# lyuchenyang/Macaw-LLM

Measured on AMD Instinct MI355X. Metric: multimodal samples/sec (img+audio+128 tok) fwd+bwd at 1/2/4/8 MI355X, higher is better.
Workload: dtype bf16; 1 GPU; BASELINE cfg 3: CLIP-ViT-L/14 + Whisper-base + LLaMA-7B, image + 30 s audio + 128-token text (S=144); fwd+bwd+fused AdamW, encoders frozen as run_clm_llms.py:390-393, alignment-attention dropout on; global_batch=32, per_gpu_batch=32, seq_len=144, parallelism=dp1: 20 flat buckets, 13476 MiB of parameters, local (one fused AdamW launch), step_launch=eager, kernel by kernel, grad_weight_side_stream=off (engine.DW_SIDE auto), setup_steps=1, activation_checkpointing=False

## Files before the change

macaw_llm_amd/build.py:

```python
from __future__ import annotations

import hashlib
import os
import shutil
import subprocess
import sys
from concurrent.futures import ThreadPoolExecutor
from pathlib import Path

PKG = Path(__file__).resolve().parent
CSRC = PKG / "csrc"
OBJ = PKG / "csrc" / "_obj"
LIB = PKG / "libmacaw_hip.so"
ARCH = "gfx950"
EXPERIMENTS = bool(os.environ.get("MK_EXPERIMENTS"))
SOURCES = ["gemm.hip", "gemm_v7.hip", *(["gemm_v8.hip"] if EXPERIMENTS else []), "gemm_v9.hip", "norm.hip",
           "elementwise.hip", "softmax.hip", "attention.hip", "decode.hip", "decode_fp8.hip", "decode_mxfp4.hip", "sample.hip", "logits_process.hip", "beam.hip", "spec.hip", "logprobs.hip", "cfg.hip", "preprocess.hip", "lora.hip"]
FLAGS = ["-O3", "-std=c++17", "-fPIC", f"--offload-arch={ARCH}", "-fno-gpu-rdc", *os.environ.get("MK_EXTRA_FLAGS", "").split(),
         *(["-DMK_WITH_V8", "-DMK_WITH_FWD4X64"] if EXPERIMENTS else []), "-Wno-unused-result"]


FILE_FLAGS = {"gemm_v8.hip": ["-mllvm", "-pragma-unroll-threshold=1000000"],
              "gemm_v9.hip": ["-mllvm", "-pragma-unroll-threshold=1000000"]}


def _hipcc() -> str:
    for cand in (os.environ.get("HIPCC"), shutil.which("hipcc"), "/opt/rocm/bin/hipcc"):
        if cand and Path(cand).exists():
            return cand
    raise RuntimeError("hipcc not found: cannot build libmacaw_hip.so")


def _digest(paths) -> str:
    h = hashlib.sha256()
    for p in sorted(paths):
        h.update(p.name.encode())
        h.update(p.read_bytes())
    h.update(" ".join(FLAGS).encode())
    h.update(repr(sorted(FILE_FLAGS.items())).encode())
    return h.hexdigest()


def build(force: bool = False, verbose: bool = True) -> Path:
    srcs = [CSRC / s for s in SOURCES]
    deps = srcs + [CSRC / "common.h", CSRC / "gemm_common.h", CSRC / "gemm_group_plan.h", PKG.parent / "include" / "macaw_hip.h",
                   *sorted(CSRC.glob("*.inc"))]
    stamp = OBJ / "stamp.txt"
    dig = _digest(deps)
    if not force and LIB.exists() and stamp.exists() and stamp.read_text() == dig:
        return LIB
    OBJ.mkdir(parents=True, exist_ok=True)
    hipcc = _hipcc()

    def compile_one(src: Path) -> Path:
        obj = OBJ / (src.stem + ".o")
        cmd = [hipcc, *FLAGS, *FILE_FLAGS.get(src.name, []), "-c", str(src), "-o", str(obj)]
        r = subprocess.run(cmd, capture_output=True, text=True)
        if r.returncode != 0:
            raise RuntimeError(f"hipcc failed for {src.name}:\n{r.stderr[-4000:]}")
        return obj

    with ThreadPoolExecutor(max_workers=min(8, len(srcs))) as ex:
        objs = list(ex.map(compile_one, srcs))
    cmd = [hipcc, "-shared", "-fPIC", f"--offload-arch={ARCH}", "-o", str(LIB), *map(str, objs)]
    r = subprocess.run(cmd, capture_output=True, text=True)
    if r.returncode != 0:
        raise RuntimeError(f"link failed:\n{r.stderr[-4000:]}")
    stamp.write_text(dig)
    if verbose:
        print(f"[macaw_llm_amd.build] built {LIB} ({LIB.stat().st_size/1e6:.1f} MB)", file=sys.stderr)
    return LIB


if __name__ == "__main__":
    build(force="--force" in sys.argv)
```

macaw_llm_amd/csrc/gemm.hip:

```cpp
#include "common.h"
#include "../../include/macaw_hip.h"
#include "gemm_common.h"
#include "gemm_group_plan.h"
#include <cstdio>
#include <algorithm>
#include <cstdlib>
#include <utility>
#include <vector>

namespace {
using namespace mkg;

constexpr int BM = 128, BN = 128, BK = 64;
#ifndef MK_GEMM_DEFAULT_CFG
#define MK_GEMM_DEFAULT_CFG 5
#endif
constexpr int TILE_BYTES = 128 * 64 * 2;
}

#define MK_E16_T bf16
#define MK_E16_NS e_bf16
#include "gemm_impl.inc"
#undef MK_E16_T
#undef MK_E16_NS
#define MK_E16_T _Float16
#define MK_E16_NS e_f16
#define gemm_bf16_kernel gemm_f16_kernel
#define gemm_bf16_v2_kernel gemm_f16_v2_kernel
#define gemm_fp8_v2_kernel gemm_fp8_v2_kernel_unused
#include "gemm_impl.inc"
#undef gemm_bf16_kernel
#undef gemm_bf16_v2_kernel
#undef gemm_fp8_v2_kernel
#undef MK_E16_T
#undef MK_E16_NS

namespace {
using namespace mkg;

constexpr int FBM = 64, FBN = 64, FBK = 16, FPAD = 4;

template <bool RED_MAJOR>
MK_DEV void f32_tile_load(const float* base, long ld, int row0, int k0, int R, int K,
                          float (*lds)[FBM + FPAD]) {
  const int t = threadIdx.x;
  if constexpr (!RED_MAJOR) {
    const int row = t >> 2, kq = (t & 3) * 4;
    const int gr = row0 + row;
#pragma unroll
    for (int j = 0; j < 4; ++j) {
      const int gk = k0 + kq + j;
      lds[kq + j][row] = (gr < R && gk < K) ? base[(long)gr * ld + gk] : 0.f;
    }
  } else {
    const int kr = t >> 4, mq = (t & 15) * 4;
    const int gk = k0 + kr;
// ... 177 lines not shown
  return N >= 8192 ? 22 : 19;
}
}

extern "C" int mk_gemm_set_cfg(int cfg) { g_force_cfg = cfg; return MK_OK; }
extern "C" int mk_gemm_has_cfg(int cfg) {
#ifdef MK_WITH_V8
  if (cfg == 14) return 1;
#endif
  return cfg == 0 || cfg == 5 || cfg == 7 || cfg == 11 || cfg == 15;
}
namespace { int g_plan_cus = 0; }
extern "C" int mk_gemm_set_cus(int n) { const int prev = g_plan_cus; g_plan_cus = n > 0 ? n : 0; return prev; }

namespace mkg {
int launch_v7(const GemmArgs& g, bool a_red, bool b_red, dim3 grid, hipStream_t st, bool fp8, bool f16);
#ifdef MK_WITH_V8
int launch_v8(const GemmArgs& g, bool a_red, bool b_red, dim3 grid, hipStream_t st, bool f16);
#endif
int launch_v9(const GemmArgs& g, bool a_red, bool b_red, dim3 grid, hipStream_t st, bool f16);
int v9_mfma16_layouts();
int launch_grp(const GrpArgs& g, bool has_main, int n_wg, hipStream_t st, bool f16);
}

extern "C" int mk_decode_linear(const void* x, int64_t ldx, const void* W, int64_t ldw, void* y,
                                int64_t ldy, const void* residual, int64_t ldr, int32_t M, int32_t N,
                                int32_t K, int32_t prologue, const void* norm_w, float eps,
                                int32_t dtype, void* stream) {
  if (!x || !W || !y || M <= 0 || N <= 0 || K <= 0) return MK_ERR_BAD_ARG;
  if (prologue < 0 || prologue > 2 || (prologue == 1 && !norm_w)) return MK_ERR_BAD_ARG;
  if ((dtype != MK_BF16 && dtype != MK_F16) || M > (prologue ? 16 : 32) || (K % 64) || (ldx % 8) || (ldw % 8) ||
      !aligned16(x) || !aligned16(W) || (prologue == 1 && !aligned16(norm_w)))
    return MK_ERR_UNSUPPORTED;
  GemmArgs g{};
  g.A = x; g.B = W; g.C = y; g.R = residual;
  g.M = M; g.N = N; g.K = K;
  g.lda = ldx; g.ldb = ldw; g.ldc = ldy; g.ldr = ldr;
  g.alpha = 1.f;
  g.pro_w = norm_w; g.pro_eps = eps;
  hipStream_t st = reinterpret_cast<hipStream_t>(stream);
  const bool wide = N <= 16 * 256 && K <= 4096;
  const size_t lds = prologue ? (size_t)M * (K + 8) * 2 : 0;
  if (lds > 40 * 1024) return MK_ERR_UNSUPPORTED;
  const int prof = mkp::begin(st, 0, 2.0 * M * N * K, M, N, K, 1, 0, 17 + 10 * prologue);
  if (M > 16) {
    if (dtype == MK_F16) e_f16::launch_skinny(g, skinny32_cfg(N), N, st);
    else e_bf16::launch_skinny(g, skinny32_cfg(N), N, st);
  } else if (dtype == MK_F16) e_f16::launch_decode_linear(g, N, prologue, wide, lds, st);
  else e_bf16::launch_decode_linear(g, N, prologue, wide, lds, st);
  mkp::end(prof, st);
  return mk_check_launch();
}
namespace {
int pick_cfg(const mk_gemm_desc* d, int nbatch, bool v7_ok, int n_cus) {
  static const bool no_v7 = getenv("MK_GEMM_NO_V7") != nullptr;
  if (!v7_ok || no_v7 || nbatch != 1) return MK_GEMM_DEFAULT_CFG;
  const int layout = (d->a_red_major ? 2 : 0) + (d->b_red_major ? 1 : 0);
  const double nk = (d->K + 63) / 64;
  const long T7 = (long)mk_cdiv(d->M, 256) * mk_cdiv(d->N, 256);
  const long full = T7 / n_cus, R = T7 % n_cus;
  const double a7 = layout == 3 ? 1.53 : layout == 1 ? 1.51 : layout == 2 ? 1.52 : 1.46;
  const double tile7 = nk * a7 + 11.5, sub7 = nk * 0.48 + 7.0;
  double t7 = full * tile7;
  if (R > 0) t7 += (4 * R <= 2 * n_cus) ? (double)mk_cdiv((int)(4 * R), n_cus) * sub7
                                         : nk * a7 * (0.55 + 0.45 * R / n_cus) + 11.5;
  const long T2 = (long)mk_cdiv(d->M, 128) * mk_cdiv(d->N, 128);
  const long slots2 = (long)n_cus * (layout == 3 ? 4 : 2);
  const double tile2 = layout == 3 ? nk * 2.18 + 4.0 : nk * (layout == 0 ? 1.67 : 1.45) + 2.0;
  const double a2 = layout == 3 ? 2.18 : layout == 0 ? 1.67 : 1.45;
  const double nk2 = layout == 3 ? 2 * nk : nk;
  double t2;
  if (T2 < slots2) {
    double sp = (double)(slots2 / T2);
    if (sp > nk2 / 2) sp = nk2 / 2;
    if (sp > 64) sp = 64;
    if (sp < 1) sp = 1;
    const double alone = sp > 1 ? 1.0 : 0.57 + 0.43 * std::min(1.0, std::max(0.0, (double)T2 / n_cus - 1.0));
    t2 = nk / sp * a2 * alone + 2.0 + (sp > 1 ? 4.0 + 1.6 * sp : 0.0);
  } else {
    t2 = (double)T2 / slots2 * tile2;
    if (const long R2 = T2 % slots2) {
      double sp = (double)slots2 / R2;
      if (sp > nk2 / 2) sp = nk2 / 2;
      if (sp > 64) sp = 64;
      t2 += 4.0 + 0.65 * sp;
    }
  }
  if (!(t7 * 0.95 < t2)) return MK_GEMM_DEFAULT_CFG;
  static const int v9_mode = [] { const char* e = getenv("MK_GEMM_V9"); return e ? atoi(e) : 1; }();
  const bool m16 = ((mkg::v9_mfma16_layouts() >> layout) & 1) != 0;
  const bool v9_legal = d->dtype != MK_F32 && d->dtype != MK_FP8 && d->M % 256 == 0 && d->N % 256 == 0 && d->K % 64 == 0 &&
                        full >= 1 && !d->scale_a && !d->scale_b &&
                        d->bias_mode == 0 && d->act == 0 && !d->accumulate && (m16 || !d->R);
  const bool nt16 = m16 && layout == 0 && !(R > 0 && full < 2 && nk < 128);
  if (v9_legal && (v9_mode == 2 || (v9_mode == 1 && (layout == 3 || layout == 1 || nk >= 256 || nt16)))) return 15;
  return 11;
}
}

extern "C" int mk_abi_version(void) { return MK_ABI_VERSION; }

extern "C" int mk_gemm(const mk_gemm_desc* d_in, void* stream) {
  const mk_gemm_desc* d = d_in;
  if (!d || !d->A || !d->B || !d->C) return MK_ERR_BAD_ARG;
  if (d->M <= 0 || d->N <= 0 || d->K <= 0) return MK_ERR_BAD_ARG;
  if (d->nb1 < 1 || d->nb2 < 1) return MK_ERR_BAD_ARG;
  if (d->bias_mode && !d->bias) return MK_ERR_BAD_ARG;
  mk_gemm_desc dd;
  bool fp8 = false;
  if (d->dtype == MK_FP8) {
    if (d->a_red_major || d->b_red_major || (d->K % 128) || (d->lda % 16) || (d->ldb % 16) ||
        (d->sA1 % 16) || (d->sA2 % 16) || (d->sB1 % 16) || (d->sB2 % 16) || !aligned16(d->A) ||
        !aligned16(d->B))
      return MK_ERR_UNSUPPORTED;
    dd = *d;
    dd.K /= 2; dd.lda /= 2; dd.ldb /= 2;
    dd.sA1 /= 2; dd.sA2 /= 2; dd.sB1 /= 2; dd.sB2 /= 2;
    dd.dtype = MK_BF16;
    d = &dd;
    fp8 = true;
  }
  if (d->dtype != MK_F32 && d->dtype != MK_BF16 && d->dtype != MK_F16) return MK_ERR_UNSUPPORTED;
  const bool f16 = d->dtype == MK_F16;
  const bool e16 = d->dtype == MK_BF16 || f16;
  GemmArgs g;
  g.scale_a = d->scale_a; g.scale_b = d->scale_b;
  g.scale_vec = (d->flags & MK_GEMM_SCALE_VEC) ? 1 : 0;
  if (g.scale_vec && (!d->scale_a || !d->scale_b)) return MK_ERR_BAD_ARG;
  if (g.scale_vec && !fp8) return MK_ERR_UNSUPPORTED;
  g.A = d->A; g.B = d->B; g.C = d->C; g.R = d->R; g.bias = d->bias;
  g.M = d->M; g.N = d->N; g.K = d->K;
  g.lda = d->lda; g.ldb = d->ldb; g.ldc = d->ldc; g.ldr = d->ldr;
  g.nb2 = d->nb2;
  g.sA1 = d->sA1; g.sA2 = d->sA2; g.sB1 = d->sB1; g.sB2 = d->sB2;
  g.sC1 = d->sC1; g.sC2 = d->sC2; g.sR1 = d->sR1; g.sR2 = d->sR2;
  g.alpha = d->alpha; g.bias_mode = d->bias_mode; g.act = d->act; g.accumulate = d->accumulate;
  hipStream_t st = reinterpret_cast<hipStream_t>(stream);
  const int nbatch = d->nb1 * d->nb2;
  const int prof = mkp::begin(st, fp8 ? 3 : 0, 2.0 * d->M * d->N * d->K * nbatch * (fp8 ? 2 : 1), d->M, d->N,
                              d->K * (fp8 ? 2 : 1), nbatch, d->a_red_major * 2 + d->b_red_major, -1);
  static const int skinny_max = [] { const char* e = getenv("MK_GEMM_SKINNY_MAX_M"); return e ? atoi(e) : 32; }();
  if (e16 && !fp8 && d->M <= 32 && d->M <= skinny_max && !d->a_red_major && !d->b_red_major && nbatch == 1 &&
      (d->K % 64) == 0 && (d->lda % 8) == 0 && (d->ldb % 8) == 0 && aligned16(d->A) && aligned16(d->B) &&
      !getenv("MK_GEMM_NO_SKINNY")) {
    int sk = d->M <= 16 ? ((d->N <= 16 * 256 && d->K <= 4096) ? 18 : 17) : skinny32_cfg(d->N);
    if ((g_force_cfg == 12 || g_force_cfg == 19 || g_force_cfg == 22) ||
        ((g_force_cfg == 13 || g_force_cfg == 17 || g_force_cfg == 18) && d->M <= 16)) sk = g_force_cfg;
// ... 28 lines not shown
      (void)hipGetDevice(&dev);
      (void)hipDeviceGetAttribute(&cus, hipDeviceAttributeMultiprocessorCount, dev);
      return cus;
    }();
    const int n_cus = (g_plan_cus > 0 && g_plan_cus < dev_cus) ? g_plan_cus : dev_cus;
    int cfg;
    if (env_cfg >= 0) cfg = env_cfg;
    else cfg = pick_cfg(d, nbatch, v7_ok, n_cus);
    if (fp8 && cfg != 11) cfg = 5;
#ifndef MK_WITH_V8
    if (cfg == 14) cfg = 11;
#endif
    if ((cfg == 11 || cfg == 14 || cfg == 15) && !v7_ok) cfg = 5;
    if ((cfg == 14 || cfg == 15) && fp8) cfg = 11;
    if (cfg == 15 && (d->M % 256 != 0 || d->N % 256 != 0 || d->K % 64 != 0 || d->K < 128)) cfg = 11;
    if (cfg == 15 && ((mkg::v9_mfma16_layouts() >> ((d->a_red_major ? 2 : 0) + (d->b_red_major ? 1 : 0))) & 1) &&
        (d->bias_mode != 0 || d->act != 0 || d->accumulate || d->scale_a || d->scale_b))
      cfg = 11;
    if (cfg != 0 && cfg != 5 && cfg != 7 && cfg != 11 && cfg != 14 && cfg != 15) cfg = 5;
    if (cfg >= 5 && !v2_ok) cfg = 0;
    if (fp8 && cfg != 5 && cfg != 11) return MK_ERR_UNSUPPORTED;
    if (cfg == 5 && d->a_red_major && d->b_red_major && !getenv("MK_GEMM_NO_BK32")) cfg = 7;
    const int bkv = cfg == 7 ? 32 : BK;
    mkp::set_cfg(prof, cfg);
    const bool v8 = cfg == 14;
    const bool v9 = cfg == 15;
    const bool t256 = cfg == 11 || v8 || v9;
    const int bm = t256 ? 256 : 128;
    const int bn = t256 ? 256 : BN;
    g.tiles_m = mk_cdiv(d->M, bm);
    g.tiles_n = mk_cdiv(d->N, bn);
    g.a_vec = aligned16(d->A) && (d->lda % 8 == 0) && (d->sA1 % 8 == 0) && (d->sA2 % 8 == 0);
    g.b_vec = aligned16(d->B) && (d->ldb % 8 == 0) && (d->sB1 % 8 == 0) && (d->sB2 % 8 == 0);
    const auto c_aligned = [&](uintptr_t mask, long q) {
      return ((reinterpret_cast<uintptr_t>(d->C) & mask) == 0) && (d->ldc % q == 0) && (d->sC1 % q == 0) &&
             (d->sC2 % q == 0) &&
             (!d->R || (((reinterpret_cast<uintptr_t>(d->R) & mask) == 0) && (d->ldr % q == 0) &&
                        (d->sR1 % q == 0) && (d->sR2 % q == 0)));
    };
    g.c_vec = c_aligned(15, 8) ? 2 : c_aligned(7, 4) ? 1 : 0;
    dim3 grid(g.tiles_m * g.tiles_n, 1, nbatch);
    g.dp_tiles = g.tiles_m * g.tiles_n;
    g.lin_batch = 0;
    g.split = 1;
    g.kt_per_piece = 0;
    g.ws = nullptr;
    g.counters = nullptr;
    g.ablate = 0;
    {
      static const int v9_lds_epi = getenv("MK_V9_LDS_EPI") ? 1 : 0;
      if (cfg == 15 && v9_lds_epi) g.ablate = 9;
    }
    g.tail8 = 0;
    const int slots = n_cus * (t256 ? 1 : (cfg == 7 ? 4 : 2));
    static const bool no_streamk = getenv("MK_GEMM_NO_STREAMK") != nullptr;
    if (t256 && !v8 && !no_streamk) {
      const int T = g.tiles_m * g.tiles_n, R = T % n_cus;
      static const bool no_tail8 = getenv("MK_GEMM_NO_TAIL8") != nullptr;
      if (R > 0 && 8 * R <= n_cus && !d->a_red_major && !no_tail8) {
        g.dp_tiles = T - R;
        g.tail8 = 1;
        grid.x = g.dp_tiles + 8 * R;
      } else if (R > 0 && 4 * R <= 2 * n_cus) {
        g.dp_tiles = T - R;
        grid.x = g.dp_tiles + 4 * R;
      }
    } else if ((cfg == 5 || cfg == 7) && d->ws && !no_streamk) {
      const int T = g.tiles_m * g.tiles_n * nbatch, nkt = (d->K + bkv - 1) / bkv;
      const int R = T % slots;
      int sp = R > 0 ? slots / R : 1;
      if (sp > nkt / 2) sp = nkt / 2;
      if (sp > 64) sp = 64;
      const long need = 4096 + (long)R * sp * (64 * 256) * 4;
      if (R > 0 && sp >= 2 && need <= d->ws_bytes) {
        g.dp_tiles = T - R;
        g.split = sp;
        g.kt_per_piece = (nkt + sp - 1) / sp;
        g.counters = reinterpret_cast<int*>(d->ws);
        g.ws = reinterpret_cast<float*>(reinterpret_cast<char*>(d->ws) + 4096);
        if (R * (int)sizeof(int) > 4096) { g.dp_tiles = T; g.split = 1; }
        else {
          grid.x = g.dp_tiles + R * sp;
          if (nbatch > 1) { g.lin_batch = 1; grid.z = 1; }
        }
      }
    }
    g.walkers = g.dp_tiles;
    if (t256 && !v8 && !v9) {
      static const bool no_walk = getenv("MK_GEMM_NO_WALK") != nullptr;
      if (!no_walk && nbatch == 1 && n_cus % 8 == 0 && g.dp_tiles > n_cus && g.dp_tiles % n_cus == 0) {
        grid.x = n_cus + (grid.x - g.dp_tiles);
        g.walkers = n_cus;
      }
    }
#ifdef MK_WITH_V8
    if (v8) {
      const int rc = mkg::launch_v8(g, d->a_red_major != 0, d->b_red_major != 0, grid, st, f16);
      mkp::end(prof, st);
      return rc;
    }
#endif
    const bool v9_c_ok = !((mkg::v9_mfma16_layouts() >> ((d->a_red_major ? 2 : 0) + (d->b_red_major ? 1 : 0))) & 1) || g.c_vec >= 1;
    if (v9 && g.dp_tiles >= n_cus && v9_c_ok) {
      const int tail_wgs = (int)grid.x - g.walkers;
      dim3 gmain(g.dp_tiles, 1, nbatch);
      static const bool no_walk9 = getenv("MK_GEMM_NO_WALK") != nullptr;
      const bool plain9 = d->bias_mode == 0 && d->act == 0 && !d->R && !d->accumulate && g.c_vec == 2 && !d->scale_a &&
                          !d->scale_b && g.ablate != 9;
      const int lay9 = (d->a_red_major ? 2 : 0) + (d->b_red_major ? 1 : 0);
      const bool regepi9 = plain9 || (((mkg::v9_mfma16_layouts() >> lay9) & 1) && g.c_vec >= 1 && d->bias_mode == 0 && d->act == 0 &&
                                      !d->accumulate && !d->scale_a && !d->scale_b && g.ablate != 9);
      if (!no_walk9 && regepi9 && nbatch == 1 && n_cus % 8 == 0 && g.dp_tiles > n_cus && g.dp_tiles % n_cus == 0)
        gmain.x = n_cus;
      int rc = mkg::launch_v9(g, d->a_red_major != 0, d->b_red_major != 0, gmain, st, f16);
      if (rc == MK_OK && tail_wgs > 0) {
        GemmArgs gt = g;
        gt.walkers = 0;
        rc = mkg::launch_v7(gt, d->a_red_major != 0, d->b_red_major != 0, dim3(tail_wgs, 1, nbatch), st, false, f16);
      }
      mkp::end(prof, st);
      return rc;
    }
    if (t256) {
      if (v9) mkp::set_cfg(prof, 11);
      const int rc = mkg::launch_v7(g, d->a_red_major != 0, d->b_red_major != 0, grid, st, fp8, f16);
      mkp::end(prof, st);
      return rc;
    }
    if (f16) (void)e_f16::launch_tile(g, cfg, d->a_red_major != 0, d->b_red_major != 0, false, grid, st);
    else (void)e_bf16::launch_tile(g, cfg, d->a_red_major != 0, d->b_red_major != 0, fp8, grid, st);
  } else {
    g.tiles_m = mk_cdiv(d->M, FBM);
    g.tiles_n = mk_cdiv(d->N, FBN);
    g.a_vec = g.b_vec = g.c_vec = 0;
    dim3 grid(g.tiles_m * g.tiles_n, 1, nbatch), block(256);
    if (!d->a_red_major && !d->b_red_major)
      MK_LAUNCH((gemm_f32_kernel<false, false>), grid, block, 0, st, g);
    else if (!d->a_red_major && d->b_red_major)
      MK_LAUNCH((gemm_f32_kernel<false, true>), grid, block, 0, st, g);
    else if (d->a_red_major && !d->b_red_major)
      MK_LAUNCH((gemm_f32_kernel<true, false>), grid, block, 0, st, g);
    else
      MK_LAUNCH((gemm_f32_kernel<true, true>), grid, block, 0, st, g);
  }
  mkp::end(prof, st);
  return mk_check_launch();
}

extern "C" int mk_gemm_grouped(const mk_gemm_desc* main, mk_gemm_group_fill* fill, int32_t n_fill, int32_t drain,
                               void* stream) {
  static_assert(mkgp::MAX_FILL == GRP_MAX_FILL && mkgp::MAX_WG == GRP_MAX_WG && MK_GROUP_MAX_FILL == GRP_MAX_FILL, "one limit");
  if (n_fill < 0 || (n_fill > 0 && !fill)) return MK_ERR_BAD_ARG;
  for (int i = 0; i < n_fill; ++i) fill[i].taken = 0;
  if (!main && n_fill == 0) return MK_OK;
  if (n_fill > GRP_MAX_FILL || mkg::v9_mfma16_layouts() != 15) return MK_NOT_GROUPED;
  const int dtype = main ? main->dtype : fill[0].d.dtype;
  if (dtype != MK_BF16 && dtype != MK_F16) return MK_NOT_GROUPED;
  const auto member = [&](const mk_gemm_desc& d, int a_red) {
    if (!d.A || !d.B || !d.C || d.M <= 0 || d.N <= 0 || d.K <= 0) return MK_ERR_BAD_ARG;
    const auto span = [&](bool red, long ld) { return red ? (long)d.K * ld * 2 : (256L * ld + d.K) * 2; };
    const bool ok = d.dtype == dtype && d.a_red_major == a_red && d.b_red_major == 1 && d.nb1 == 1 && d.nb2 == 1 &&
                    d.M % 256 == 0 && d.N % 256 == 0 && d.K % 64 == 0 && d.K >= 128 && d.bias_mode == 0 && !d.bias && d.act == 0 &&
                    !d.R && !d.accumulate && !d.scale_a && !d.scale_b && d.flags == 0 && aligned16(d.A) && aligned16(d.B) &&
                    d.lda % 8 == 0 && d.ldb % 8 == 0 && (reinterpret_cast<uintptr_t>(d.C) & 7) == 0 && d.ldc % 4 == 0 &&
                    d.lda >= (a_red ? d.M : d.K) && d.ldb >= d.N && d.ldc >= d.N &&
                    span(a_red != 0, d.lda) < 0x7fffffffL && span(true, d.ldb) < 0x7fffffffL;
// ... 71 lines not shown
```

macaw_llm_amd/csrc/gemm_common.h:

```cpp
#pragma once
#include "common.h"
#include "../../include/macaw_hip.h"

namespace mkg {

struct GemmArgs {
  const void* A; const void* B; void* C; const void* R; const void* bias;
  int M, N, K;
  long lda, ldb, ldc, ldr;
  int nb2;
  long sA1, sA2, sB1, sB2, sC1, sC2, sR1, sR2;
  float alpha;
  const float* scale_a; const float* scale_b;
  int scale_vec;
  int bias_mode, act, accumulate;
  int tiles_m, tiles_n;
  int a_vec, b_vec;
  int c_vec;
  int dp_tiles, split, kt_per_piece;
  int walkers;
  int tail8;
  int lin_batch;
  int ablate;
  const void* pro_w; float pro_eps;
  float* ws;
  int* counters;
};

constexpr int GRP_MAX_FILL = 8, GRP_MAX_WG = 320;
struct GrpProb {
  const void* A; const void* B; void* C;
  long lda, ldb, ldc;
  int M, N, K;
  int tiles_m, tiles_n;
  int first, count;
  float alpha;
};
struct GrpArgs {
  GrpProb p[1 + GRP_MAX_FILL];
  int n_fill;
  int main_tiles;
  unsigned short start[GRP_MAX_WG + 1];
};

MK_DEV float apply_act(float v, int act) {
  if (act == 1) return 0.5f * v * (1.0f + mk_erf(v * 0.70710678118654752440f));
  if (act == 2) return v / (1.0f + __expf(-1.702f * v));
  return v;
}

MK_DEV int xcd_remap(int bid, int nwg) {
  const int xcd = bid & 7;
  const int q = nwg >> 3, r = nwg & 7;
  return (xcd < r ? xcd * (q + 1) : r * (q + 1) + (xcd - r) * q) + (bid >> 3);
}
MK_DEV void tile_from_index(int wg, int tiles_m, int tiles_n, int& tm, int& tn, int GROUP_M);
MK_DEV void tile_coords(int bid, int tiles_m, int tiles_n, int& tm, int& tn) {
  tile_from_index(xcd_remap(bid, tiles_m * tiles_n), tiles_m, tiles_n, tm, tn, 8);
}
MK_DEV void tile_from_index(int wg, int tiles_m, int tiles_n, int& tm, int& tn, int GROUP_M = 8) {
  const int per_group = GROUP_M * tiles_n;
  const int group = wg / per_group;
  const int first_m = group * GROUP_M;
  const int gsize = min(tiles_m - first_m, GROUP_M);
  const int in_g = wg - group * per_group;
  tm = first_m + in_g % gsize;
  tn = in_g / gsize;
}

template <bool SV, typename ET, int FM, int FN>
MK_DEV void wave_epilogue(const f32x16 (&acc)[FM][FN], const GemmArgs& g, ET* C, const ET* Rp,
                          int m0, int n0, int wm0, int wn0, char* smem) {
  typedef typename E16<ET>::x4 e16x4;
  constexpr int W4 = FN * 8;
// ... 249 lines not shown
```

macaw_llm_amd/csrc/gemm_v9.hip:

```cpp
#include "gemm_common.h"
#include "gemm_v9_loop.inc"

#define MK_E16_T bf16
#define MK_E16_NS e_bf16
#define MK_V9_SFX "bf16"
#include "gemm_v9_impl.inc"
#undef MK_E16_T
#undef MK_E16_NS
#undef MK_V9_SFX
#define MK_E16_T _Float16
#define MK_E16_NS e_f16
#define MK_V9_SFX "f16"
#define gemm_bf16_v9_kernel gemm_f16_v9_kernel
#define gemm_bf16_grp_kernel gemm_f16_grp_kernel
#include "gemm_v9_impl.inc"
#undef gemm_bf16_v9_kernel
#undef gemm_bf16_grp_kernel
#undef MK_E16_T
#undef MK_E16_NS
#undef MK_V9_SFX

namespace mkg {
int v9_mfma16_layouts() {
#ifdef V9_MFMA16
  return V9_MFMA16;
#else
  return 0;
#endif
}
int launch_v9(const GemmArgs& g, bool a_red, bool b_red, dim3 grid, hipStream_t st, bool f16) {
  if (f16) {
    if (!a_red && !b_red) return e_f16::launch_v9<false, false>(g, grid, st);
    if (!a_red && b_red) return e_f16::launch_v9<false, true>(g, grid, st);
    if (a_red && !b_red) return e_f16::launch_v9<true, false>(g, grid, st);
    return e_f16::launch_v9<true, true>(g, grid, st);
  }
  if (!a_red && !b_red) return e_bf16::launch_v9<false, false>(g, grid, st);
  if (!a_red && b_red) return e_bf16::launch_v9<false, true>(g, grid, st);
  if (a_red && !b_red) return e_bf16::launch_v9<true, false>(g, grid, st);
  return e_bf16::launch_v9<true, true>(g, grid, st);
}
int launch_grp(const GrpArgs& g, bool has_main, int n_wg, hipStream_t st, bool f16) {
  return f16 ? e_f16::launch_grp(g, has_main, n_wg, st) : e_bf16::launch_grp(g, has_main, n_wg, st);
}
}
```

macaw_llm_amd/csrc/gemm_v9_impl.inc:

```

namespace {
namespace MK_E16_NS {
using namespace mkg;
typedef MK_E16_T e16;
typedef E16<e16>::x8 e16x8;
typedef E16<e16>::x4 e16x4;

constexpr int BM9 = 256, BN9 = 256, BK7 = 64;
constexpr int HALF_BYTES = 128 * BK7 * 2;
constexpr int A_SLOT = 2 * HALF_BYTES;
constexpr int B_BASE9 = 3 * A_SLOT;
constexpr int LDS9 = 5 * A_SLOT;

#include "gemm_lds_image.inc"

typedef uint32_t u32x4 __attribute__((ext_vector_type(4)));

struct V9Tile {
  int m0, n0;
  e16* C;
  const e16* Rp;
  __amdgpu_buffer_rsrc_t rsA, rsB;
  u32x4 dA, dB;
  int voA[2][4], voB[2][4];
// ... 46 lines not shown
  t.dA[3] = 0x00020000u;
  t.dB[0] = __builtin_amdgcn_readfirstlane((uint32_t)pb);
  t.dB[1] = __builtin_amdgcn_readfirstlane((uint32_t)(pb >> 32) & 0xffffu);
  t.dB[2] = (uint32_t)b_rec;
  t.dB[3] = 0x00020000u;
#pragma unroll
  for (int h = 0; h < 2; ++h)
#pragma unroll
    for (int i = 0; i < 4; ++i) {
      t.voA[h][i] = v9_voffset<A_RED, M16>(m0, g.M, g.lda, h, w + 4 * i, l);
      t.voB[h][i] = v9_voffset<B_RED, M16>(n0, g.N, g.ldb, h, w + 4 * i, l);
    }
}

template <typename T>
MK_DEV T* v9_batch_elem(T* p, long z1, long s1, long z2, long s2) {
  return p + z1 * s1 + z2 * s2;
}
template <bool A_RED, bool B_RED>
MK_DEV void v9_tile_setup(const GemmArgs& g, int tile, int w, int l, V9Tile& t) {
  int tm, tn;
  tile_from_index(xcd_remap(tile, g.dp_tiles), g.tiles_m, g.tiles_n, tm, tn, 8);
  const int z = blockIdx.z, z1 = z / g.nb2, z2 = z - z1 * g.nb2;
  const e16* A = v9_batch_elem(reinterpret_cast<const e16*>(g.A), z1, g.sA1, z2, g.sA2);
  const e16* B = v9_batch_elem(reinterpret_cast<const e16*>(g.B), z1, g.sB1, z2, g.sB2);
  t.C = v9_batch_elem(reinterpret_cast<e16*>(g.C), z1, g.sC1, z2, g.sC2);
  t.Rp = g.R ? v9_batch_elem(reinterpret_cast<const e16*>(g.R), z1, g.sR1, z2, g.sR2) : nullptr;
  v9_operand_setup<A_RED, B_RED, true>(g, A, B, tm * BM9, tn * BN9, w, l, t);
}

MK_DEV void v9_tile_request(const V9Tile& t, char* smem, int w, int stepA, int stepB) {
#define V9_DMA_A(DST, H, I, KO)                                                                   \
  __builtin_amdgcn_raw_ptr_buffer_load_lds(                                                       \
      t.rsA, (__attribute__((address_space(3))) void*)(smem + (DST) + (H) * HALF_BYTES + (w + 4 * (I)) * 1024), \
      16, t.voA[H][I], KO, 0, 0)
#define V9_DMA_B(DST, H, I, KO)                                                                   \
  __builtin_amdgcn_raw_ptr_buffer_load_lds(                                                       \
      t.rsB, (__attribute__((address_space(3))) void*)(smem + (DST) + (H) * HALF_BYTES + (w + 4 * (I)) * 1024), \
      16, t.voB[H][I], KO, 0, 0)
#pragma unroll
  for (int h = 0; h < 2; ++h)
#pragma unroll
    for (int i = 0; i < 4; ++i) { V9_DMA_A(0, h, i, 0); V9_DMA_B(B_BASE9, h, i, 0); }
#pragma unroll
  for (int h = 0; h < 2; ++h)
#pragma unroll
    for (int i = 0; i < 4; ++i) V9_DMA_A(A_SLOT, h, i, stepA);
#pragma unroll
  for (int i = 0; i < 4; ++i) V9_DMA_B(B_BASE9 + A_SLOT, 0, i, stepB);
#undef V9_DMA_A
#undef V9_DMA_B
}

#define V9_ASM(TEXT, CLOBBERS)                                                                    \
  asm volatile(TEXT                                                                               \
               :                                                                                  \
               : [voA] "v"(t.voA[0][0]), [voB] "v"(t.voB[0][0]), [adA] "v"(adA), [adB] "v"(adB),   \
                 [rsA] "s"(t.dA), [rsB] "s"(t.dB), [iA] "s"(iA), [iB] "s"(iB), [stA] "s"(stepA),   \
                 [stB] "s"(stepB), [nk] "s"(nk), [wv] "s"(wv)                                      \
               : CLOBBERS)
#if V9_MFMA16
#ifdef MK_V9_NT_STORE
typedef unsigned int v9_u32x2 __attribute__((ext_vector_type(2)));
#define V9_ST8(PTR, VAL) __builtin_nontemporal_store(__builtin_bit_cast(v9_u32x2, VAL), reinterpret_cast<v9_u32x2*>(PTR))
#else
#define V9_ST8(PTR, VAL) (*reinterpret_cast<e16x4*>(PTR) = (VAL))
#endif
#define V9_F16P(I, J, CROW, LDC, ALPHA)                                           \
  do {                                                                                            \
    float t_[4];                                                                                  \
    V9_ACC16_READ_##I##_##J(t_);                                                                  \
    e16x4 o_;                                                                                     \
    _Pragma("unroll") for (int e_ = 0; e_ < 4; ++e_) o_[e_] = (e16)(t_[e_] * (ALPHA));           \
    V9_ST8((CROW) + (long)(16 * (I)) * (LDC) + 16 * (J), o_);                                     \
  } while (0)
#define V9_R16(F, I, CROW, LDC, ALPHA)                                                            \
  do {                                                                                            \
    F(I, 0, CROW, LDC, ALPHA); F(I, 1, CROW, LDC, ALPHA); F(I, 2, CROW, LDC, ALPHA); F(I, 3, CROW, LDC, ALPHA); \
    F(I, 4, CROW, LDC, ALPHA); F(I, 5, CROW, LDC, ALPHA); F(I, 6, CROW, LDC, ALPHA); F(I, 7, CROW, LDC, ALPHA); \
    __builtin_amdgcn_sched_barrier(0);                                                            \
  } while (0)
#define V9_EPI16(F, CROW, LDC, ALPHA)                                                             \
  do {                                                                                            \
    V9_R16(F, 0, CROW, LDC, ALPHA); V9_R16(F, 1, CROW, LDC, ALPHA); V9_R16(F, 2, CROW, LDC, ALPHA); \
    V9_R16(F, 3, CROW, LDC, ALPHA); V9_R16(F, 4, CROW, LDC, ALPHA); V9_R16(F, 5, CROW, LDC, ALPHA); \
    V9_R16(F, 6, CROW, LDC, ALPHA); V9_R16(F, 7, CROW, LDC, ALPHA);                               \
  } while (0)
#endif

template <bool A_RED, bool B_RED>
__global__ __launch_bounds__(256, 1) void gemm_bf16_v9_kernel(GemmArgs g) {
  extern __shared__ __attribute__((aligned(16))) char smem[];
  const int l = threadIdx.x & 63;
  const int w = __builtin_amdgcn_readfirstlane(threadIdx.x >> 6);
  const int wr = w >> 1, wc = w & 1;
  const int wm0 = wr * 128, wn0 = wc * 128;
  const int stepA = A_RED ? (int)(BK7 * g.lda * 2) : BK7 * 2;
  const int stepB = B_RED ? (int)(BK7 * g.ldb * 2) : BK7 * 2;
  const int iA = (int)((A_RED ? 16 : 32) * g.lda * 2);
  const int iB = (int)((B_RED ? 16 : 32) * g.ldb * 2);
  int offA[4], offB[4];
  v7_read_offsets<A_RED>(0, l, offA);
  v7_read_offsets<B_RED>(0, l, offB);
  const int nk = __builtin_amdgcn_readfirstlane((g.K + BK7 - 1) / BK7);
  const uint32_t lds0 = __builtin_amdgcn_readfirstlane(
      (uint32_t)(size_t)((__attribute__((address_space(3))) char*)smem));
  const uint32_t wv = lds0 + (uint32_t)w * 1024u;
  constexpr bool M16 = ((V9_MFMA16 >> (2 * (A_RED ? 1 : 0) + (B_RED ? 1 : 0))) & 1) != 0;
  const uint32_t adA = lds0 + wr * HALF_BYTES + (M16 ? v9_read_offset16<A_RED>(l) : offA[0]);
  const uint32_t adB = lds0 + B_BASE9 + wc * HALF_BYTES + (M16 ? v9_read_offset16<B_RED>(l) : offB[0]);
  const bool plain = g.bias_mode == 0 && g.act == 0 && g.R == nullptr && g.accumulate == 0 && (g.c_vec == 2 || (M16 && g.c_vec >= 1)) &&
                     g.scale_a == nullptr && g.scale_b == nullptr && g.ablate != 9;

  int tile = blockIdx.x;
  const int stride = (int)gridDim.x;
  V9Tile t;
  v9_tile_setup<A_RED, B_RED>(g, tile, w, l, t);
  v9_tile_request(t, smem, w, stepA, stepB);
  bool first = true;
  for (;;) {
    __builtin_amdgcn_sched_barrier(0);
#define V9_LOOPS(W)                                                                               \
  do {                                                                                            \
    if constexpr (!A_RED && !B_RED) V9_ASM(V9_LOOP_TEXT_00##W, V9_LOOP_CLOBBERS);                 \
    else if constexpr (!A_RED && B_RED) V9_ASM(V9_LOOP_TEXT_01##W, V9_LOOP_CLOBBERS);             \
    else if constexpr (A_RED && !B_RED) V9_ASM(V9_LOOP_TEXT_10##W, V9_LOOP_CLOBBERS);             \
    else V9_ASM(V9_LOOP_TEXT_11##W, V9_LOOP_CLOBBERS);                                            \
  } while (0)
#if V9_MFMA16
#define V9_LOOPS16(W)                                                                             \
  do {                                                                                            \
    if constexpr (!A_RED && !B_RED) V9_ASM(V9_LOOP16_TEXT_00##W, V9_LOOP16_CLOBBERS);             \
    else if constexpr (!A_RED && B_RED) V9_ASM(V9_LOOP16_TEXT_01##W, V9_LOOP16_CLOBBERS);         \
    else if constexpr (A_RED && !B_RED) V9_ASM(V9_LOOP16_TEXT_10##W, V9_LOOP16_CLOBBERS);         \
    else V9_ASM(V9_LOOP16_TEXT_11##W, V9_LOOP16_CLOBBERS);                                        \
  } while (0)
    if constexpr (M16) {
      if (first) V9_LOOPS16();
      else V9_LOOPS16(_W);
    } else
#endif
    {
      if (first) V9_LOOPS();
      else V9_LOOPS(_W);
    }
#undef V9_LOOPS
#undef V9_LOOPS16
    __builtin_amdgcn_sched_barrier(0);
#ifdef MK_V9_NOEPI
    return;
#endif
    const int m0 = t.m0, n0 = t.n0;
    e16* C = t.C;
    const e16* Rp = t.Rp;
    const int ntile = tile + stride;
    const bool more = ntile < g.dp_tiles;
    if (more) {
      v9_tile_setup<A_RED, B_RED>(g, ntile, w, l, t);
      __builtin_amdgcn_s_barrier();
      v9_tile_request(t, smem, w, stepA, stepB);
    }
#if V9_MFMA16
    if constexpr (M16) {
      const float alpha = g.alpha;
      const int mrow = m0 + wm0 + (l & 15), ncol = n0 + wn0 + 4 * (l >> 4);
      e16* crow = C + (long)mrow * g.ldc + ncol;
      const e16* rrow = Rp ? Rp + (long)mrow * g.ldr + ncol : nullptr;
#define V9_F16R(I, J, CROW, LDC, ALPHA)    \
  do {                                                                                            \
    float t_[4];                                                                                  \
    V9_ACC16_READ_##I##_##J(t_);                                                                  \
    e16x4 o_;                                                                                     \
    _Pragma("unroll") for (int e_ = 0; e_ < 4; ++e_) o_[e_] = (e16)(t_[e_] * (ALPHA) + (float)rv_[I][J][e_]); \
    V9_ST8((CROW) + (long)(16 * (I)) * (LDC) + 16 * (J), o_);                                     \
  } while (0)
      if (rrow == nullptr) {
        V9_EPI16(V9_F16P, crow, g.ldc, alpha);
      } else {
        e16x4 rv_[8][8];
#pragma unroll
        for (int i_ = 0; i_ < 8; ++i_)
#pragma unroll
          for (int j_ = 0; j_ < 8; ++j_)
            rv_[i_][j_] = *reinterpret_cast<const e16x4*>(rrow + (long)(16 * i_) * g.ldr + 16 * j_);
        __builtin_amdgcn_sched_barrier(0);
        V9_EPI16(V9_F16R, crow, g.ldc, alpha);
      }
#undef V9_F16R
    } else
#endif
    if (plain) {
      const int half = l >> 5;
      const float alpha = g.alpha;
      e16* crow = C + (long)(m0 + wm0 + (l & 31)) * g.ldc + n0 + wn0 + 8 * half;
#define V9_FRAG(I, J)                                                                             \
  do {                                                                                            \
    float t_[16];                                                                                 \
    V9_ACC_READ_##I##_##J(t_);                                                                    \
    e16* rp_ = crow + (long)(32 * (I)) * g.ldc + 32 * (J);                                        \
    _Pragma("unroll") for (int p_ = 0; p_ < 2; ++p_) {                                            \
      e16x4 lo_, hi_;                                                                             \
      _Pragma("unroll") for (int e_ = 0; e_ < 4; ++e_) {                                          \
        lo_[e_] = (e16)(t_[8 * p_ + e_] * alpha);                                                 \
        hi_[e_] = (e16)(t_[8 * p_ + 4 + e_] * alpha);                                             \
      }                                                                                           \
      const uint2 a_ = __builtin_bit_cast(uint2, lo_), b_ = __builtin_bit_cast(uint2, hi_);       \
      const auto sx_ = __builtin_amdgcn_permlane32_swap(a_.x, b_.x, false, false);                \
      const auto sy_ = __builtin_amdgcn_permlane32_swap(a_.y, b_.y, false, false);                \
      u32x4 o_;                                                                                   \
      o_[0] = sx_[0]; o_[1] = sy_[0]; o_[2] = sx_[1]; o_[3] = sy_[1];                             \
      *reinterpret_cast<u32x4*>(rp_ + 16 * p_) = o_;                                              \
    }                                                                                             \
  } while (0)
#define V9_FROW(I) V9_FRAG(I, 0); V9_FRAG(I, 1); V9_FRAG(I, 2); V9_FRAG(I, 3)
      V9_FROW(0); V9_FROW(1); V9_FROW(2); V9_FROW(3);
#undef V9_FROW
#undef V9_FRAG
    } else {
#define V9_ROW(I)                                                                                 \
  do {                                                                                            \
    float t0_[16], t1_[16], t2_[16], t3_[16];                                                     \
    V9_ACC_READ_##I##_0(t0_); V9_ACC_READ_##I##_1(t1_); V9_ACC_READ_##I##_2(t2_); V9_ACC_READ_##I##_3(t3_); \
    f32x16 r_[1][4];                                                                              \
    _Pragma("unroll") for (int e_ = 0; e_ < 16; ++e_) {                                           \
      r_[0][0][e_] = t0_[e_]; r_[0][1][e_] = t1_[e_]; r_[0][2][e_] = t2_[e_]; r_[0][3][e_] = t3_[e_]; \
    }                                                                                             \
    wave_epilogue16<false, e16, 1, 4>(r_, g, C, Rp, m0, n0, wm0 + 32 * (I), wn0, smem, (I) == 0); \
  } while (0)
      V9_ROW(0);
      V9_ROW(1);
      V9_ROW(2);
      V9_ROW(3);
#undef V9_ROW
    }
    if (!more) break;
    tile = ntile;
    first = false;
  }
}

#if V9_MFMA16 == 15
template <bool A_RED>
MK_DEV void grp_tile_setup(const GrpProb& p, int lin, int w, int l, V9Tile& t) {
  int tm, tn;
  tile_from_index(lin, p.tiles_m, p.tiles_n, tm, tn, 8);
  t.C = reinterpret_cast<e16*>(p.C);
  t.Rp = nullptr;
  v9_operand_setup<A_RED, true, false>(p, reinterpret_cast<const e16*>(p.A), reinterpret_cast<const e16*>(p.B), tm * BM9,
                                       tn * BN9, w, l, t);
}

struct GrpCursor {
  int mt, stride;
  int j, cnt, base;
  int cl;
  uint64_t below;
};
template <bool HAS_MAIN>
MK_DEV bool grp_next(const GrpArgs& g, GrpCursor& c, int& pi, int& lin) {
  if (HAS_MAIN && c.mt < g.main_tiles) {
    pi = 0;
    lin = xcd_remap(c.mt, g.main_tiles);
    c.mt += c.stride;
    return true;
  }
  if (c.j >= c.cnt) return false;
  const uint64_t act = __builtin_amdgcn_ballot_w64(c.cl > c.j);
  int at = c.base + __builtin_popcountll(act & c.below), f = 1;
  c.base += __builtin_popcountll(act);
  ++c.j;
  while (f < g.n_fill && at >= g.p[f].count) at -= g.p[f++].count;
  pi = f;
  lin = g.p[f].first + at;
  return true;
}

template <bool HAS_MAIN>
__global__ __launch_bounds__(256, 1) void gemm_bf16_grp_kernel(GrpArgs g) {
  extern __shared__ __attribute__((aligned(16))) char smem[];
  const int l = threadIdx.x & 63;
  const int w = __builtin_amdgcn_readfirstlane(threadIdx.x >> 6);
  const int wr = w >> 1, wc = w & 1;
  const int wm0 = wr * 128, wn0 = wc * 128;
  const uint32_t lds0 = __builtin_amdgcn_readfirstlane(
      (uint32_t)(size_t)((__attribute__((address_space(3))) char*)smem));
  const uint32_t wv = lds0 + (uint32_t)w * 1024u;
  const uint32_t adA_k = lds0 + wr * HALF_BYTES + v9_read_offset16<false>(l);
  const uint32_t adA_r = lds0 + wr * HALF_BYTES + v9_read_offset16<true>(l);
  const uint32_t adB = lds0 + B_BASE9 + wc * HALF_BYTES + v9_read_offset16<true>(l);
  const int n = (int)gridDim.x, b = (int)blockIdx.x;
// ... 97 lines not shown
```

Measured before the change: 151.1 samples/s.

## Process v9 GEMM wave-quantization tail as sub-tile pieces inside the persistent launch

When the 256x256 tile count leaves a remainder that is not a multiple of the CU count, the v9 persistent kernel now splits each leftover tile into eight 64x128 pieces. Persistent blocks pick these pieces up after their last full tile, using an XCD-aware piece assignment, instead of relying on a separate tail launch or the stream-K path. This targets the idle CUs in the last partial wave and the extra launch overhead for mid-K GEMMs. It also widens the NT layout heuristic so that such shapes choose cfg 15. The cost is a new hand-scheduled MFMA loop with its own inline asm and waitcnt logic, which adds correctness and register-pressure risk.

```diff
diff --git a/macaw_llm_amd/build.py b/macaw_llm_amd/build.py
--- a/macaw_llm_amd/build.py
+++ b/macaw_llm_amd/build.py
@@ -43,7 +43,7 @@
 
 def build(force: bool = False, verbose: bool = True) -> Path:
     srcs = [CSRC / s for s in SOURCES]
-    deps = srcs + [CSRC / "common.h", CSRC / "gemm_common.h", CSRC / "gemm_group_plan.h", PKG.parent / "include" / "macaw_hip.h",
+    deps = srcs + [CSRC / "common.h", CSRC / "gemm_common.h", CSRC / "gemm_group_plan.h", CSRC / "gemm_tail_plan.h", PKG.parent / "include" / "macaw_hip.h",
                    *sorted(CSRC.glob("*.inc"))]
     stamp = OBJ / "stamp.txt"
     dig = _digest(deps)
diff --git a/macaw_llm_amd/csrc/gemm.hip b/macaw_llm_amd/csrc/gemm.hip
--- a/macaw_llm_amd/csrc/gemm.hip
+++ b/macaw_llm_amd/csrc/gemm.hip
@@ -2,6 +2,7 @@
 #include "../../include/macaw_hip.h"
 #include "gemm_common.h"
 #include "gemm_group_plan.h"
+#include "gemm_tail_plan.h"
 #include <cstdio>
 #include <algorithm>
 #include <cstdlib>
@@ -285,6 +286,13 @@
   return mk_check_launch();
 }
 namespace {
+constexpr int V9_TAIL_MAX_PIECES = 1, V9_TAIL_MAX_NK = 96;
+bool v9_tail_in_launch(int n_cus, long T, long nk) {
+  static const int mode = [] { const char* e = getenv("MK_GEMM_V9_TAIL"); return e ? atoi(e) : 1; }();
+  const int R = (int)(T % n_cus);
+  if (mode == 0 || n_cus % 8 != 0 || R == 0 || T - R < n_cus) return false;
+  return mode == 2 || (nk <= V9_TAIL_MAX_NK && mktp::tail_max_pieces(n_cus, R) <= V9_TAIL_MAX_PIECES);
+}
 int pick_cfg(const mk_gemm_desc* d, int nbatch, bool v7_ok, int n_cus) {
   static const bool no_v7 = getenv("MK_GEMM_NO_V7") != nullptr;
   if (!v7_ok || no_v7 || nbatch != 1) return MK_GEMM_DEFAULT_CFG;
@@ -325,7 +333,7 @@
   const bool v9_legal = d->dtype != MK_F32 && d->dtype != MK_FP8 && d->M % 256 == 0 && d->N % 256 == 0 && d->K % 64 == 0 &&
                         full >= 1 && !d->scale_a && !d->scale_b &&
                         d->bias_mode == 0 && d->act == 0 && !d->accumulate && (m16 || !d->R);
-  const bool nt16 = m16 && layout == 0 && !(R > 0 && full < 2 && nk < 128);
+  const bool nt16 = m16 && layout == 0 && (!(R > 0 && full < 2 && nk < 128) || v9_tail_in_launch(n_cus, T7, (long)nk));
   if (v9_legal && (v9_mode == 2 || (v9_mode == 1 && (layout == 3 || layout == 1 || nk >= 256 || nt16)))) return 15;
   return 11;
 }
@@ -460,6 +468,7 @@
       if (cfg == 15 && v9_lds_epi) g.ablate = 9;
     }
     g.tail8 = 0;
+    g.tail_r = 0;
     const int slots = n_cus * (t256 ? 1 : (cfg == 7 ? 4 : 2));
     static const bool no_streamk = getenv("MK_GEMM_NO_STREAMK") != nullptr;
     if (t256 && !v8 && !no_streamk) {
@@ -520,6 +529,18 @@
                                       !d->accumulate && !d->scale_a && !d->scale_b && g.ablate != 9);
       if (!no_walk9 && regepi9 && nbatch == 1 && n_cus % 8 == 0 && g.dp_tiles > n_cus && g.dp_tiles % n_cus == 0)
         gmain.x = n_cus;
+      const int T9 = g.tiles_m * g.tiles_n, R9 = T9 % n_cus;
+      if (v9_tail_in_launch(n_cus, T9, d->K / 64) && !no_streamk && !no_walk9 && regepi9 &&
+          ((mkg::v9_mfma16_layouts() >> lay9) & 1) && !d->a_red_major && nbatch == 1) {
+        g.dp_tiles = T9 - R9;
+        g.walkers = g.dp_tiles;
+        g.tail8 = 0;
+        g.tail_r = R9;
+        gmain.x = n_cus;
+        const int rc1 = mkg::launch_v9(g, false, d->b_red_major != 0, gmain, st, f16);
+        mkp::end(prof, st);
+        return rc1;
+      }
       int rc = mkg::launch_v9(g, d->a_red_major != 0, d->b_red_major != 0, gmain, st, f16);
       if (rc == MK_OK && tail_wgs > 0) {
         GemmArgs gt = g;
diff --git a/macaw_llm_amd/csrc/gemm_common.h b/macaw_llm_amd/csrc/gemm_common.h
--- a/macaw_llm_amd/csrc/gemm_common.h
+++ b/macaw_llm_amd/csrc/gemm_common.h
@@ -20,6 +20,7 @@
   int dp_tiles, split, kt_per_piece;
   int walkers;
   int tail8;
+  int tail_r;
   int lin_batch;
   int ablate;
   const void* pro_w; float pro_eps;
diff --git a/macaw_llm_amd/csrc/gemm_tail_plan.h b/macaw_llm_amd/csrc/gemm_tail_plan.h
--- /dev/null
+++ b/macaw_llm_amd/csrc/gemm_tail_plan.h
@@ -0,0 +1,34 @@
+#pragma once
+
+#if defined(__HIPCC__) || defined(__CUDACC__)
+#define MK_TP_FN __host__ __device__ inline
+#else
+#define MK_TP_FN inline
+#endif
+
+namespace mktp {
+
+MK_TP_FN bool tail_xcd_form(int n, int R) {
+  if (n < 8 || (n & 7) != 0 || R < 1) return false;
+  if ((R & 7) == 0) return true;
+  const int w = n >> 3, a = R >> 3;
+  const int lo = 8 * a / w, hi = (8 * (a + 1) + w - 1) / w;
+  return hi - lo <= 1;
+}
+
+MK_TP_FN int tail_max_pieces(int n, int R) { return n > 0 && R > 0 ? (8 * R + n - 1) / n : 0; }
+
+MK_TP_FN int tail_piece(int b, int n, int R, int j) {
+  if (b < 0 || b >= n || R < 1 || j < 0) return -1;
+  if (!tail_xcd_form(n, R)) {
+    const long p = (long)j * n + b;
+    return p < 8L * R ? (int)p : -1;
+  }
+  const int x = b & 7, k = b >> 3, w = n >> 3;
+  const int tiles = (R - x + 7) >> 3;
+  const long q = (long)j * w + k;
+  if (q >= 8L * tiles) return -1;
+  return (int)(8 * (x + 8 * (q >> 3)) + (q & 7));
+}
+
+}
diff --git a/macaw_llm_amd/csrc/gemm_v9.hip b/macaw_llm_amd/csrc/gemm_v9.hip
--- a/macaw_llm_amd/csrc/gemm_v9.hip
+++ b/macaw_llm_amd/csrc/gemm_v9.hip
@@ -1,4 +1,5 @@
 #include "gemm_common.h"
+#include "gemm_tail_plan.h"
 #include "gemm_v9_loop.inc"
 
 #define MK_E16_T bf16
diff --git a/macaw_llm_amd/csrc/gemm_v9_impl.inc b/macaw_llm_amd/csrc/gemm_v9_impl.inc
--- a/macaw_llm_amd/csrc/gemm_v9_impl.inc
+++ b/macaw_llm_amd/csrc/gemm_v9_impl.inc
@@ -122,6 +122,176 @@
 #undef V9_DMA_B
 }
 
+struct V9Piece {
+  int m0, n0;
+  __amdgpu_buffer_rsrc_t rsA, rsB;
+  int voA[2], voB[4];
+};
+template <bool B_RED>
+MK_DEV void v9_piece_setup(const GemmArgs& g, int piece, int w, int l, V9Piece& p) {
+  int tm, tn;
+  tile_from_index(g.dp_tiles + (piece >> 3), g.tiles_m, g.tiles_n, tm, tn, 8);
+  const int m0 = tm * BM9 + ((piece >> 1) & 3) * 64, n0 = tn * BN9 + (piece & 1) * 128;
+  p.m0 = m0; p.n0 = n0;
+  const e16* A = reinterpret_cast<const e16*>(g.A);
+  const e16* B = reinterpret_cast<const e16*>(g.B);
+  const e16* abase = uniform_ptr(A + (long)m0 * g.lda);
+  const e16* bbase = uniform_ptr(B_RED ? B + n0 : B + (long)n0 * g.ldb);
+  const long a_bytes = ((long)(min(g.M - m0, 64) - 1) * g.lda + ((g.K + 1) & ~1)) * 2;
+  const long b_bytes = B_RED ? ((long)(g.K - 1) * g.ldb + ((g.N - n0 + 1) & ~1)) * 2
+                             : ((long)(min(g.N - n0, 128) - 1) * g.ldb + ((g.K + 1) & ~1)) * 2;
+  p.rsA = __builtin_amdgcn_make_buffer_rsrc(
+      (void*)abase, 0, __builtin_amdgcn_readfirstlane((int)min(a_bytes, 0x7fffffffL)), 0x00020000);
+  p.rsB = __builtin_amdgcn_make_buffer_rsrc(
+      (void*)bbase, 0, __builtin_amdgcn_readfirstlane((int)min(b_bytes, 0x7fffffffL)), 0x00020000);
+#pragma unroll
+  for (int i = 0; i < 2; ++i) p.voA[i] = v7_voffset<false>(m0, g.M, g.lda, 0, w + 4 * i, l);
+#pragma unroll
+  for (int i = 0; i < 4; ++i) p.voB[i] = v7_voffset<B_RED>(n0, g.N, g.ldb, 0, w + 4 * i, l);
+}
+MK_DEV void v9_piece_issue(const V9Piece& p, char* smem, int w, int st, int kA, int kB) {
+  char* dst = smem + st * A_SLOT + w * 1024;
+#pragma unroll
+  for (int i = 0; i < 2; ++i)
+    __builtin_amdgcn_raw_ptr_buffer_load_lds(
+        p.rsA, (__attribute__((address_space(3))) void*)(dst + i * 4096), 16, p.voA[i], kA, 0, 0);
+#pragma unroll
+  for (int i = 0; i < 4; ++i)
+    __builtin_amdgcn_raw_ptr_buffer_load_lds(
+        p.rsB, (__attribute__((address_space(3))) void*)(dst + HALF_BYTES + i * 4096), 16, p.voB[i], kB, 0, 0);
+}
+MK_DEV void v9_piece_request(const V9Piece& p, char* smem, int w, int nk, int stepA, int stepB) {
+#pragma unroll 1
+  for (int s = 0; s < 4 && s < nk; ++s) v9_piece_issue(p, smem, w, s, s * stepA, s * stepB);
+}
+template <bool B_RED>
+MK_DEV void v9_tail_pieces(const GemmArgs& g, V9Piece& p, int piece, int b, int n, char* smem, int w, int l, int nk,
+                           int stepA, int stepB) {
+  const int wm0 = (w >> 1) * 32, wn0 = (w & 1) * 64;
+  int offA[4], offB[4];
+  v7_read_offsets<false>(wm0, l, offA);
+  v7_read_offsets<B_RED>(wn0, l, offB);
+  e16* const C = reinterpret_cast<e16*>(g.C);
+  const e16* const Rp = reinterpret_cast<const e16*>(g.R);
+  const float alpha = g.alpha;
+#define V9T_WAIT(AHEAD)                                                        \
+  do {                                                                         \
+    if ((AHEAD) >= 2) asm volatile("s_waitcnt vmcnt(12)" ::: "memory");        \
+    else if ((AHEAD) == 1) asm volatile("s_waitcnt vmcnt(6)" ::: "memory");    \
+    else asm volatile("s_waitcnt vmcnt(0)" ::: "memory");                      \
+    __builtin_amdgcn_sched_barrier(0);                                         \
+    __builtin_amdgcn_s_barrier();                                              \
+    __builtin_amdgcn_sched_barrier(0);                                         \
+  } while (0)
+#define V9T_READ(FA, FB, ST)                                                   \
+  do {                                                                         \
+    int aad[4], bad[4];                                                        \
+    _Pragma("unroll") for (int i = 0; i < 4; ++i) {                            \
+      aad[i] = (ST) * A_SLOT + offA[i];                                        \
+      bad[i] = (ST) * A_SLOT + HALF_BYTES + offB[i];                           \
+    }                                                                          \
+    _Pragma("unroll") for (int ks = 0; ks < 4; ++ks) {                         \
+      FB[0][ks] = V7_FRAG(B_RED, bad, 0, ks);                                  \
+      FB[1][ks] = V7_FRAG(B_RED, bad, 1, ks);                                  \
+      FA[ks] = V7_FRAG(false, aad, 0, ks);                                     \
+    }                                                                          \
+  } while (0)
+#define V9T_MFMA(ACC, B_, A_) "v_mfma_f32_32x32x16_" MK_V9_SFX " " ACC ", " B_ ", " A_ ", " ACC "\n\t"
+#define V9T_DRAIN() asm volatile("s_nop 7" : "+v"(acc[0]), "+v"(acc[1]))
+#define V9T_MMA(FA, FB)                                                      \
+  do {                                                                         \
+    asm volatile("s_nop 1\n\t" V9T_MFMA("%0", "%2", "%10") V9T_MFMA("%1", "%6", "%10")                         \
+                 V9T_MFMA("%0", "%3", "%11") V9T_MFMA("%1", "%7", "%11") V9T_MFMA("%0", "%4", "%12")              \
+                 V9T_MFMA("%1", "%8", "%12") V9T_MFMA("%0", "%5", "%13") V9T_MFMA("%1", "%9", "%13")              \
+                 "s_nop 15\n\ts_nop 3"                                                                            \
+                 : "+v"(acc[0]), "+v"(acc[1])                                                                     \
+                 : "v"(FB[0][0]), "v"(FB[0][1]), "v"(FB[0][2]), "v"(FB[0][3]), "v"(FB[1][0]), "v"(FB[1][1]),     \
+                   "v"(FB[1][2]), "v"(FB[1][3]), "v"(FA[0]), "v"(FA[1]), "v"(FA[2]), "v"(FA[3]));                \
+  } while (0)
+#define V9T_STEP(FX, BX, FY, BY)                                               \
+  do {                                                                         \
+    if (t + 1 < nk) {                                                          \
+      V9T_WAIT(nk - 2 - t);                                                    \
+      V9T_READ(FY, BY, st1);                                                   \
+    }                                                                          \
+    V9T_MMA(FX, BX);                                                           \
+    if (t + 4 < nk) {                                                          \
+      v9_piece_issue(p, smem, w, st_in, kA, kB);                               \
+      kA += stepA; kB += stepB;                                                \
+      st_in = st_in == 4 ? 0 : st_in + 1;                                      \
+    }                                                                          \
+    st1 = st1 == 4 ? 0 : st1 + 1;                                              \
+    ++t;                                                                       \
+  } while (0)
+  for (int j = 0;;) {
+    const int m0 = p.m0, n0 = p.n0;
+    f32x16 acc[2];
+#pragma unroll
+    for (int e = 0; e < 16; ++e) { acc[0][e] = 0.f; acc[1][e] = 0.f; }
+    int st_in = 4, kA = 4 * stepA, kB = 4 * stepB;
+    e16x8 fa0[4], fb0[2][4], fa1[4], fb1[2][4];
+    V9T_WAIT(0);
+    V9T_READ(fa0, fb0, 0);
+    int st1 = 1, t = 0;
+    while (t < nk) {
+      V9T_STEP(fa0, fb0, fa1, fb1);
+      if (t >= nk) break;
+      V9T_STEP(fa1, fb1, fa0, fb0);
+    }
+    V9T_DRAIN();
+    piece = mktp::tail_piece(b, n, g.tail_r, ++j);
+    if (piece >= 0) {
+      v9_piece_setup<B_RED>(g, piece, w, l, p);
+      __builtin_amdgcn_sched_barrier(0);
+      __builtin_amdgcn_s_barrier();
+      __builtin_amdgcn_sched_barrier(0);
+      v9_piece_request(p, smem, w, nk, stepA, stepB);
+    }
+    {
+      const int mrow = m0 + wm0 + (l & 31), ncol = n0 + wn0 + 4 * (l >> 5);
+      e16* crow = C + (long)mrow * g.ldc + ncol;
+      if (Rp == nullptr) {
+#pragma unroll
+        for (int f = 0; f < 2; ++f)
+#pragma unroll
+          for (int q = 0; q < 4; ++q) {
+            e16x4 o_;
+#pragma unroll
+            for (int e = 0; e < 4; ++e) o_[e] = (e16)(acc[f][4 * q + e] * alpha);
+            *reinterpret_cast<e16x4*>(crow + 32 * f + 8 * q) = o_;
+          }
+      } else {
+        const e16* rrow = Rp + (long)mrow * g.ldr + ncol;
+        e16x4 rv_[2][4];
+#pragma unroll
+        for (int f = 0; f < 2; ++f)
+#pragma unroll
+          for (int q = 0; q < 4; ++q) rv_[f][q] = *reinterpret_cast<const e16x4*>(rrow + 32 * f + 8 * q);
+#pragma unroll
+        for (int f = 0; f < 2; ++f)
+#pragma unroll
+          for (int q = 0; q < 4; ++q) {
+            e16x4 o_;
+#pragma unroll
+            for (int e = 0; e < 4; ++e) {
+              float v_ = acc[f][4 * q + e] * alpha + (float)rv_[f][q][e];
+              asm volatile("" : "+v"(v_));
+              o_[e] = (e16)v_;
+            }
+            *reinterpret_cast<e16x4*>(crow + 32 * f + 8 * q) = o_;
+          }
+      }
+    }
+    if (piece < 0) break;
+  }
+#undef V9T_STEP
+#undef V9T_MMA
+#undef V9T_DRAIN
+#undef V9T_MFMA
+#undef V9T_READ
+#undef V9T_WAIT
+}
+
 #define V9_ASM(TEXT, CLOBBERS)                                                                    \
   asm volatile(TEXT                                                                               \
                :                                                                                  \
@@ -188,6 +358,9 @@
   v9_tile_setup<A_RED, B_RED>(g, tile, w, l, t);
   v9_tile_request(t, smem, w, stepA, stepB);
   bool first = true;
+  constexpr bool TAIL9 = M16 && !A_RED;
+  V9Piece pc;
+  int piece = -1;
   for (;;) {
     __builtin_amdgcn_sched_barrier(0);
 #define V9_LOOPS(W)                                                                               \
@@ -229,6 +402,13 @@
       v9_tile_setup<A_RED, B_RED>(g, ntile, w, l, t);
       __builtin_amdgcn_s_barrier();
       v9_tile_request(t, smem, w, stepA, stepB);
+    } else if constexpr (TAIL9) {
+      if (g.tail_r > 0) piece = mktp::tail_piece((int)blockIdx.x, stride, g.tail_r, 0);
+      if (piece >= 0) {
+        v9_piece_setup<B_RED>(g, piece, w, l, pc);
+        __builtin_amdgcn_s_barrier();
+        v9_piece_request(pc, smem, w, nk, stepA, stepB);
+      }
     }
 #if V9_MFMA16
     if constexpr (M16) {
@@ -306,6 +486,9 @@
     if (!more) break;
     tile = ntile;
     first = false;
+  }
+  if constexpr (TAIL9) {
+    if (piece >= 0) v9_tail_pieces<B_RED>(g, pc, piece, (int)blockIdx.x, stride, smem, w, l, nk, stepA, stepB);
   }
 }
 
```

Result: no change. 151.2 samples/s, median of 2 (+0.1%).
